# GAP-LAB-CUHK-SZ/GaussReg

Measured on AMD Instinct MI355X. Metric: GS views/sec @1M pts 640x480 (+ radius_neighbors Mpts/sec, see radius_neighbors), higher is better.
Workload: dtype f32; 1 GPU; diff_gaussian_rasterization forward: 1000000 synthetic Gaussians (SH deg 3), 640x480, 32 views per step per GPU (configs[1]); gaussians=1000000, width=640, height=480, parallelism=per-view sharding x1

## Files before the change

### gaussreg_amd/_lib.py

```python
import ctypes
import os
import re

_HERE = os.path.dirname(os.path.abspath(__file__))
LIB_PATH = os.path.join(_HERE, "lib", "libgaussreg_hip.so")
HEADER_PATH = os.path.join(_HERE, "..", "include", "gaussreg_hip.h")
TRAIN_HEADER_PATH = os.path.join(_HERE, "..", "include", "gaussreg_hip_train.h")
MATCH_TRAIN_HEADER_PATH = os.path.join(_HERE, "..", "include", "gaussreg_hip_train_matching.h")
BACKBONE_TRAIN_HEADER_PATH = os.path.join(_HERE, "..", "include", "gaussreg_hip_train_backbone.h")

_lib = None

c_void = ctypes.c_void_p
c_f32 = ctypes.c_float


class RasterView(ctypes.Structure):
    _fields_ = [("image_height", ctypes.c_int32), ("image_width", ctypes.c_int32),
                ("tanfovx", c_f32), ("tanfovy", c_f32), ("bg", c_f32 * 3), ("scale_modifier", c_f32),
                ("viewmatrix", c_f32 * 16), ("projmatrix", c_f32 * 16), ("campos", c_f32 * 3),
                ("sh_degree", ctypes.c_int32), ("prefiltered", ctypes.c_int32), ("debug", ctypes.c_int32)]


class GsAdamGroup(ctypes.Structure):
    _fields_ = [("param", c_void), ("grad", c_void), ("exp_avg", c_void), ("exp_avg_sq", c_void),
                ("lr", ctypes.c_double), ("K", ctypes.c_int32)]


class GsDensifyGroup(ctypes.Structure):
    _fields_ = [("src_param", c_void), ("dst_param", c_void), ("src_exp_avg", c_void), ("dst_exp_avg", c_void),
                ("src_exp_avg_sq", c_void), ("dst_exp_avg_sq", c_void), ("K", ctypes.c_int32), ("role", ctypes.c_int32)]

# ... 35 lines not shown
        if r is None:
            raise ValueError(f"gaussreg_hip.h: cannot parse the return type '{ret}' of {name}")
        restype = None if r.groups() == ("void", "") else _ctype(r.group(1), r.group(2), f"the return type of {name}")
        argtypes = []
        for arg in ([] if args in ("", "void") else args.split(",")):
            a = re.fullmatch(_TYPE + r"(?:\s*(\*)\s*|\s+)\w+", arg.strip())
            if a is None:
                raise ValueError(f"gaussreg_hip.h: cannot parse the argument '{arg.strip()}' of {name}")
            argtypes.append(_ctype(a.group(1), a.group(2) or "", f"argument '{arg.strip()}' of {name}"))
        if name in signatures:
            raise ValueError(f"gaussreg_hip.h: {name} is declared twice")
        signatures[name] = (restype, argtypes)
    return signatures, defines


with open(HEADER_PATH) as _f:
    SIGNATURES, DEFINES = parse_header(_f.read())
with open(TRAIN_HEADER_PATH) as _f:
    TRAIN_SIGNATURES, TRAIN_DEFINES = parse_header(_f.read())
with open(MATCH_TRAIN_HEADER_PATH) as _f:
    MATCH_TRAIN_SIGNATURES, MATCH_TRAIN_DEFINES = parse_header(_f.read())
with open(BACKBONE_TRAIN_HEADER_PATH) as _f:
    BACKBONE_TRAIN_SIGNATURES, BACKBONE_TRAIN_DEFINES = parse_header(_f.read())

GR_PENDING = DEFINES["GR_PENDING"]
GR_RETRY_FULL = DEFINES["GR_RETRY_FULL"]
GR_RETRY_BIN = DEFINES["GR_RETRY_BIN"]
GS_ADAM_MAX_GROUPS = DEFINES["GR_GS_ADAM_MAX_GROUPS"]
GS_KNN_MAX_K = DEFINES["GR_GS_KNN_MAX_K"]
GS_DENSIFY_CARRIED, GS_DENSIFY_XYZ, GS_DENSIFY_SCALING = (DEFINES["GR_GS_DENSIFY_" + r] for r in ("CARRIED", "XYZ", "SCALING"))


class HipLibraryError(RuntimeError):
    pass


def lib():
    global _lib
    if _lib is None:
        import torch
        if not os.path.exists(LIB_PATH):
            raise HipLibraryError(
                f"{LIB_PATH} is missing: build it with `python -m gaussreg_amd.build` "
                "(there is no CPU fallback for the gaussreg_amd ops)")
        L = ctypes.CDLL(LIB_PATH)
        for name, (res, args) in (list(SIGNATURES.items()) + list(TRAIN_SIGNATURES.items())
                                   + list(MATCH_TRAIN_SIGNATURES.items()) + list(BACKBONE_TRAIN_SIGNATURES.items())):
            fn = getattr(L, name)
            fn.restype = res
            fn.argtypes = args
        _lib = L
    return _lib


def check(rc, allow=()):
    if rc != 0 and rc not in allow:
        msg = lib().gr_last_error()
        raise RuntimeError("gaussreg_hip: " + (msg.decode() if msg else f"error {rc}"))
    return rc


def tensor_stamp(tensors):
    out = []
    for t in tensors:
        if t.is_inference():
            return None
        out.append((t.data_ptr(), t._version))
    return tuple(out)


# ... 87 lines not shown
```

### gaussreg_amd/build.py

```python
import concurrent.futures
import os
import subprocess
import sys

HERE = os.path.dirname(os.path.abspath(__file__))
CSRC = os.path.join(HERE, "csrc")
LIBDIR = os.path.join(HERE, "lib")
OBJDIR = os.path.join(LIBDIR, "obj")
LIB = os.path.join(LIBDIR, "libgaussreg_hip.so")

HIPCC = os.environ.get("HIPCC", "/opt/rocm/bin/hipcc")
FLAGS = ["--offload-arch=gfx950", "-O3", "-std=c++17", "-fPIC", "-ffp-contract=off", "-Wall",
         "-Wno-unused-function", "-Wno-unused-result"]


def sources():
    return sorted(f for f in os.listdir(CSRC) if f.endswith(".hip"))


def _stale(out, deps):
    if not os.path.exists(out):
        return True
    t = os.path.getmtime(out)
    return any(os.path.getmtime(d) > t for d in deps)


def build(force=False, verbose=False):
    os.makedirs(OBJDIR, exist_ok=True)
    headers = [os.path.join(CSRC, f) for f in os.listdir(CSRC) if f.endswith((".hpp", ".h"))]
    headers += [os.path.join(HERE, "..", "include", h) for h in ("gaussreg_hip.h", "gaussreg_hip_train.h",
                                                                 "gaussreg_hip_train_matching.h",
                                                                 "gaussreg_hip_train_backbone.h")]
    jobs = []
    objs = []
    for src in sources():
        s = os.path.join(CSRC, src)
        o = os.path.join(OBJDIR, src[:-4] + ".o")
        objs.append(o)
        if force or _stale(o, [s] + headers):
            jobs.append([HIPCC] + FLAGS + ["-c", s, "-o", o])

    def run(cmd):
        if verbose:
            print(" ".join(cmd), flush=True)
        r = subprocess.run(cmd, stdout=subprocess.PIPE, stderr=subprocess.STDOUT, text=True)
        return cmd, r.returncode, r.stdout

    if jobs:
        with concurrent.futures.ThreadPoolExecutor(max_workers=min(8, len(jobs))) as ex:
            for cmd, rc, out in ex.map(run, jobs):
                if rc != 0:
                    raise RuntimeError("hipcc failed: %s\n%s" % (" ".join(cmd), out))
                if verbose and out.strip():
                    print(out)
    if force or jobs or _stale(LIB, objs):
# ... 10 lines not shown
```

### gaussreg_amd/csrc/preprocess_body.hpp

```cpp
#ifndef GR_PREPROCESS_BODY_OK
#error "preprocess_body.hpp is the body of the two preprocess kernels of rasterizer.hip"
#endif
static_assert(std::is_same<decltype(WAVE_MM), const bool>::value, "the including kernel defines `constexpr bool WAVE_MM`");
  if (LATE && blockIdx.x == 0 && threadIdx.x < (int)(sizeof(DevView) / 4))
    reinterpret_cast<float*>(const_cast<DevView*>(views))[threadIdx.x] = reinterpret_cast<const float*>(&cam1)[threadIdx.x];
  __shared__ float4 s_sh[(SH16 && !LATE) ? WAVE * SH_ROW : 1];
  __shared__ float4 s_rec[256 / WAVE][4 * REC_PLANE];
  __shared__ int s_mm[WAVE_MM ? 1 : 2][2][256 / WAVE];
  int i = blockIdx.x * blockDim.x + threadIdx.x;
  float shr[SH16 ? 48 : 1];
  if (SH16 && !LATE) {
    const int g0 = blockIdx.x * 256;
    const int n_here = min(256, P - g0);
    const float4* src = reinterpret_cast<const float4*>(shs + (int64_t)g0 * 48);
#pragma unroll 1
    for (int w = 0; w < 256 / WAVE; ++w) {
      const int lim = min(WAVE, n_here - w * WAVE) * 12;
#pragma unroll
      for (int u = 0; u < 3; ++u) {
        const int f = threadIdx.x + u * 256;
        if (f < lim) {
          const int g = f / 12, j = f - g * 12;
          s_sh[g * SH_ROW + j] = src[w * WAVE * 12 + f];
        }
      }
      __syncthreads();
      if ((int)threadIdx.x / WAVE == w && i < P) {
#pragma unroll
// ... 14 lines not shown
  i = min(i, P - 1);
  const float p[3] = {means3D[3 * (int64_t)i], means3D[3 * (int64_t)i + 1], means3D[3 * (int64_t)i + 2]};
  const float opacity = opacities[i];
  float c6[6];
  if (HAS_COV) {
#pragma unroll
    for (int k = 0; k < 6; ++k) c6[k] = cov3D_precomp[6 * (int64_t)i + k];
  }
  const int gx = (W + TILE - 1) / TILE, gy = (H + TILE - 1) / TILE;
  const float* sh = HAS_SH ? shs + (int64_t)i * M * 3 : nullptr;
  float cpre[3] = {0.f, 0.f, 0.f};
  if (!HAS_SH) {
#pragma unroll
    for (int k = 0; k < 3; ++k) cpre[k] = colors_precomp[3 * (int64_t)i + k];
  }
  float4* wrec = s_rec[threadIdx.x / WAVE];
  float mod_prev = 0.f;
  bool have_cov = HAS_COV;
  for (int v = 0; v < V; ++v) {
    const DevView& cam = LATE ? cam1 : views[v];
    const int64_t o = (int64_t)v * P + i;
    int out_radius = 0;
    uint32_t out_field = 0u, out_rect = 0u;
    float out_depth = 0.f, out_sxx = INFINITY, out_syy = INFINITY, out_kc = 0.f;
    float2 out_xy = make_float2(0.f, 0.f);
    float4 out_co = make_float4(0.f, 0.f, 0.f, 0.f);
    bool shade = false;
    float rgb[3] = {0.f, 0.f, 0.f};
    float pv[3];
    xform4x3(cam.view, p, pv);
    if (pv[2] > 0.2f) {
      float ph[4];
      xform4x4(cam.proj, p, ph);
      const float pw = 1.0f / (ph[3] + 0.0000001f);
      const float pprojx = ph[0] * pw, pprojy = ph[1] * pw;
      if (!HAS_COV && (!have_cov || cam.scale_mod != mod_prev)) {
        float sc[3], rot[4];
#pragma unroll
        for (int k = 0; k < 3; ++k) sc[k] = scales[3 * (int64_t)i + k];
#pragma unroll
        for (int k = 0; k < 4; ++k) rot[k] = rotations[4 * (int64_t)i + k];
        cov3d_from_scale_rot(sc, cam.scale_mod, rot, c6);
        have_cov = true;
        mod_prev = cam.scale_mod;
      }
      float cv[3];
      cov2d(pv, cam.fx, cam.fy, cam.tanx, cam.tany, c6, cam.view, cv);
      const float det = cv[0] * cv[2] - cv[1] * cv[1];
      if (det != 0.0f) {
        const float det_inv = 1.f / det;
        const float mid = 0.5f * (cv[0] + cv[2]);
        const float sq = sqrtf(fmaxf(0.1f, mid * mid - det));
        const float l1 = mid + sq, l2 = mid - sq;
        const float my_radius = ceilf(3.f * sqrtf(fmaxf(l1, l2)));
        const float px = ((pprojx + 1.0f) * (float)W - 1.0f) * 0.5f;
        const float py = ((pprojy + 1.0f) * (float)H - 1.0f) * 0.5f;
        int rmin[2], rmax[2];
        get_rect(px, py, (int)my_radius, gx, gy, rmin, rmax);
        const int ntile = (rmax[0] - rmin[0]) * (rmax[1] - rmin[1]);
        if (ntile != 0) {
          shade = true;
          if (HAS_SH && SH16 && LATE) {
            const float4* s4 = reinterpret_cast<const float4*>(shs + (int64_t)i * 48);
#pragma unroll
            for (int jj = 0; jj < 12; ++jj) {
              const float4 t4 = s4[jj];
              shr[4 * jj] = t4.x;
              shr[4 * jj + 1] = t4.y;
              shr[4 * jj + 2] = t4.z;
              shr[4 * jj + 3] = t4.w;
            }
            sh_to_rgb(D, p, cam.campos, [&](int k, int c) { return shr[k * 3 + c]; }, rgb);
          }
          out_depth = pv[2];
          out_radius = (int)my_radius;
          out_xy = make_float2(px, py);
          out_co = make_float4(cv[2] * det_inv, -cv[1] * det_inv, cv[0] * det_inv, opacity);
          const bool cullable = det > 0.0f && l2 >= 0.29f && l1 < 1.0e4f;
          const float kc = cullable ? 1.001f / (0.5f / l1 - 2.0e-6f) : INFINITY;
          out_kc = kc;
          if (cullable) {
            out_sxx = 2.0f * cv[0] * 1.004f;
            out_syy = 2.0f * cv[2] * 1.004f;
            const float pcm = __logf(255.0f * opacity) + 2.0e-3f;
            if (pcm > 0.0f) {
              const float cp = pcm + 2.0e-6f * (pcm * kc);
              const float hx = sqrtf(2.0f * cp * cv[0]) * 1.001f + 1.0e-2f;
              const float hy = sqrtf(2.0f * cp * cv[2]) * 1.001f + 1.0e-2f;
              const float xlo = ceilf(px - hx), xhi = floorf(px + hx), ylo = ceilf(py - hy), yhi = floorf(py + hy);
              if (xlo > -1.0e6f && xhi < 1.0e6f && ylo > -1.0e6f && yhi < 1.0e6f) {
                rmin[0] = max(rmin[0], (int)floorf(xlo / (float)TILE));
                rmin[1] = max(rmin[1], (int)floorf(ylo / (float)TILE));
                rmax[0] = min(rmax[0], (int)floorf(xhi / (float)TILE) + 1);
                rmax[1] = min(rmax[1], (int)floorf(yhi / (float)TILE) + 1);
                if (rmax[0] < rmin[0]) rmax[0] = rmin[0];
                if (rmax[1] < rmin[1]) rmax[1] = rmin[1];
              }
            }
          }
          uint32_t dk = __float_as_uint(out_depth) - KEY_DEPTH_BASE;
          if (dk >= (1u << KEY_DEPTH_BITS)) {
            dk = (1u << KEY_DEPTH_BITS) - 1;
            if (LATE) *far_flag = far_seq; else atomicOr(far_flag, 1);
          }
          out_field = dk;
          out_rect = pack_rect(rmin, rmax);
        }
      }
    }
    if (valid) {
      __builtin_nontemporal_store(out_radius, radii + o);
      dfield[o] = out_field;
      rect_raw[o] = out_rect;
    }
    wrec[0 * REC_PLANE + lane] = make_float4(out_xy.x, out_xy.y, out_sxx, out_syy);
    wrec[1 * REC_PLANE + lane] = out_co;
    wrec[3 * REC_PLANE + lane] = make_float4(__int_as_float(out_radius), out_depth, 0.f, 0.f);
    if (WAVE_MM) {
      const uint32_t fld = valid ? out_field : 0u;
      const int mn = wave_min_i32_dpp(fld != 0u ? (int)fld : 0x7fffffff), mx = wave_max_i32_dpp((int)fld);
      const int wave_id = __builtin_amdgcn_readfirstlane((int)(blockIdx.x * (256 / WAVE) + threadIdx.x / WAVE));
      if (lane == 0) key_mm[(int64_t)v * (gridDim.x * (256 / WAVE)) + wave_id] = make_int2(mn, mx);
      __builtin_amdgcn_fence(__ATOMIC_RELEASE, "wavefront");
      __builtin_amdgcn_wave_barrier();
      __builtin_amdgcn_fence(__ATOMIC_ACQUIRE, "wavefront");
    } else if (key_mm != nullptr) {
      const uint32_t fld = valid ? out_field : 0u;
      const int mn = wave_min_i32_dpp(fld != 0u ? (int)fld : 0x7fffffff), mx = wave_max_i32_dpp((int)fld);
      if (lane == 0) s_mm[v & 1][0][threadIdx.x / WAVE] = mn, s_mm[v & 1][1][threadIdx.x / WAVE] = mx;
      __syncthreads();
      if (threadIdx.x == 0) {
        int bmn = 0x7fffffff, bmx = 0;
#pragma unroll
        for (int w = 0; w < 256 / WAVE; ++w) bmn = min(bmn, s_mm[v & 1][0][w]), bmx = max(bmx, s_mm[v & 1][1][w]);
        key_mm[(int64_t)v * gridDim.x + blockIdx.x] = make_int2(bmn, bmx);
      }
    }
    if (shade && !(HAS_SH && SH16 && LATE)) {
      if (HAS_SH) {
        if (SH16) sh_to_rgb(D, p, cam.campos, [&](int k, int c) { return shr[k * 3 + c]; }, rgb);
        else sh_to_rgb(D, p, cam.campos, [&](int k, int c) { return sh[k * 3 + c]; }, rgb);
      } else {
        rgb[0] = cpre[0]; rgb[1] = cpre[1]; rgb[2] = cpre[2];
      }
    }
    wrec[2 * REC_PLANE + lane] = make_float4(rgb[0], rgb[1], rgb[2], out_kc);
    const unsigned long long vis = __ballot(valid && out_radius > 0);
    __builtin_amdgcn_fence(__ATOMIC_RELEASE, "wavefront");
    __builtin_amdgcn_wave_barrier();
    __builtin_amdgcn_fence(__ATOMIC_ACQUIRE, "wavefront");
    float4* wout = rec + 4 * ((int64_t)v * P + wave_first);
#pragma unroll
    for (int k = 0; k < 4; ++k) {
      const int rl = 16 * k + lane / 4;
      const float4 piece = wrec[(lane & 3) * REC_PLANE + rl];
      if ((vis >> rl) & 1ull) {
        typedef float pre_f4 __attribute__((ext_vector_type(4)));
        __builtin_nontemporal_store(pre_f4{piece.x, piece.y, piece.z, piece.w}, reinterpret_cast<pre_f4*>(wout + 4 * rl + (lane & 3)));
      }
    }
    __builtin_amdgcn_fence(__ATOMIC_RELEASE, "wavefront");
    __builtin_amdgcn_wave_barrier();
    __builtin_amdgcn_fence(__ATOMIC_ACQUIRE, "wavefront");
  }
```

### gaussreg_amd/csrc/raster_shared.hpp

```cpp
#pragma once

#include "common.hpp"

namespace gr {
namespace {

constexpr int TILE = 16;
constexpr int BLOCK = TILE * TILE;
constexpr int MAX_VIEWS = 64;

struct DevView {
  float view[16];
  float proj[16];
  float campos[3];
  float tanx, tany;
  float fx, fy;
  float scale_mod;
  float bg[3];
};

__device__ __constant__ float SH_C0 = 0.28209479177387814f;
__device__ __constant__ float SH_C1 = 0.4886025119029199f;
__device__ __constant__ float SH_C2[5] = {1.0925484305920792f, -1.0925484305920792f,
                                          0.31539156525252005f, -1.0925484305920792f,
// ... 11 lines not shown
  const float nf = tm - MAGIC;
  const float f = fmaf(x, L2E, -nf);
  float p = 1.3264815788716078e-3f;
  p = fmaf(p, f, 9.671512059867382e-3f);
  p = fmaf(p, f, 5.550733581185341e-2f);
  p = fmaf(p, f, 2.4022242426872253e-1f);
  p = fmaf(p, f, 6.931470036506653e-1f);
  p = fmaf(p, f, 1.0f);
  return __uint_as_float(__float_as_uint(p) + (__float_as_uint(tm) << 23));
}

__device__ __forceinline__ void xform4x3(const float* M, const float* p, float* o) {
  o[0] = fmaf(M[0], p[0], fmaf(M[4], p[1], fmaf(M[8], p[2], M[12])));
  o[1] = fmaf(M[1], p[0], fmaf(M[5], p[1], fmaf(M[9], p[2], M[13])));
  o[2] = fmaf(M[2], p[0], fmaf(M[6], p[1], fmaf(M[10], p[2], M[14])));
}
__device__ __forceinline__ void xform4x4(const float* M, const float* p, float* o) {
  o[0] = fmaf(M[0], p[0], fmaf(M[4], p[1], fmaf(M[8], p[2], M[12])));
  o[1] = fmaf(M[1], p[0], fmaf(M[5], p[1], fmaf(M[9], p[2], M[13])));
  o[2] = fmaf(M[2], p[0], fmaf(M[6], p[1], fmaf(M[10], p[2], M[14])));
  o[3] = fmaf(M[3], p[0], fmaf(M[7], p[1], fmaf(M[11], p[2], M[15])));
}

__device__ __forceinline__ void cov3d_from_scale_rot(const float* sc, float mod, const float* q,
                                                     float* c6) {
  const float s0 = mod * sc[0], s1 = mod * sc[1], s2 = mod * sc[2];
  const float r = q[0], x = q[1], y = q[2], z = q[3];
  float R[3][3];
  R[0][0] = 1.f - 2.f * (y * y + z * z);
  R[0][1] = 2.f * (x * y - r * z);
  R[0][2] = 2.f * (x * z + r * y);
  R[1][0] = 2.f * (x * y + r * z);
  R[1][1] = 1.f - 2.f * (x * x + z * z);
  R[1][2] = 2.f * (y * z - r * x);
  R[2][0] = 2.f * (x * z - r * y);
  R[2][1] = 2.f * (y * z + r * x);
  R[2][2] = 1.f - 2.f * (x * x + y * y);
  float M[3][3];
#pragma unroll
  for (int i = 0; i < 3; ++i) {
    M[0][i] = s0 * R[i][0];
    M[1][i] = s1 * R[i][1];
    M[2][i] = s2 * R[i][2];
  }
#define GR_SIG(i, j) fmaf(M[0][i], M[0][j], fmaf(M[1][i], M[1][j], M[2][i] * M[2][j]))
  c6[0] = GR_SIG(0, 0);
  c6[1] = GR_SIG(0, 1);
  c6[2] = GR_SIG(0, 2);
  c6[3] = GR_SIG(1, 1);
  c6[4] = GR_SIG(1, 2);
  c6[5] = GR_SIG(2, 2);
#undef GR_SIG
}

__device__ __forceinline__ void cov2d(const float* t_in, float fx, float fy, float tanx, float tany,
                                      const float* c6, const float* V, float* out3) {
  float t[3] = {t_in[0], t_in[1], t_in[2]};
  const float limx = 1.3f * tanx, limy = 1.3f * tany;
  const float txtz = t[0] / t[2], tytz = t[1] / t[2];
  t[0] = fminf(limx, fmaxf(-limx, txtz)) * t[2];
  t[1] = fminf(limy, fmaxf(-limy, tytz)) * t[2];
  const float J00 = fx / t[2];
  const float J02 = -(fx * t[0]) / (t[2] * t[2]);
  const float J11 = fy / t[2];
  const float J12 = -(fy * t[1]) / (t[2] * t[2]);
  float A0[3], A1[3];
#pragma unroll
  for (int j = 0; j < 3; ++j) {
    A0[j] = fmaf(J00, V[j * 4 + 0], J02 * V[j * 4 + 2]);
    A1[j] = fmaf(J11, V[j * 4 + 1], J12 * V[j * 4 + 2]);
  }
  const float S[3][3] = {{c6[0], c6[1], c6[2]}, {c6[1], c6[3], c6[4]}, {c6[2], c6[4], c6[5]}};
  float B0[3], B1[3];
#pragma unroll
  for (int k = 0; k < 3; ++k) {
    B0[k] = fmaf(S[k][0], A0[0], fmaf(S[k][1], A0[1], S[k][2] * A0[2]));
    B1[k] = fmaf(S[k][0], A1[0], fmaf(S[k][1], A1[1], S[k][2] * A1[2]));
  }
  out3[0] = fmaf(A0[0], B0[0], fmaf(A0[1], B0[1], A0[2] * B0[2])) + 0.3f;
  out3[1] = fmaf(A1[0], B0[0], fmaf(A1[1], B0[1], A1[2] * B0[2]));
  out3[2] = fmaf(A1[0], B1[0], fmaf(A1[1], B1[1], A1[2] * B1[2])) + 0.3f;
}

template <typename ShLoad>
__device__ __forceinline__ void sh_to_rgb(int deg, const float* pos, const float* campos,
                                          ShLoad S, float* rgb) {
  const float dx = pos[0] - campos[0], dy = pos[1] - campos[1], dz = pos[2] - campos[2];
  const float len = sqrtf(dx * dx + dy * dy + dz * dz);
  const float x = dx / len, y = dy / len, z = dz / len;
#pragma unroll
  for (int c = 0; c < 3; ++c) {
    float res = SH_C0 * S(0, c);
    if (deg > 0) {
      res = res - SH_C1 * y * S(1, c) + SH_C1 * z * S(2, c) - SH_C1 * x * S(3, c);
      if (deg > 1) {
        const float xx = x * x, yy = y * y, zz = z * z, xy = x * y, yz = y * z, xz = x * z;
        res = res + SH_C2[0] * xy * S(4, c) + SH_C2[1] * yz * S(5, c) +
              SH_C2[2] * (2.0f * zz - xx - yy) * S(6, c) + SH_C2[3] * xz * S(7, c) +
              SH_C2[4] * (xx - yy) * S(8, c);
        if (deg > 2) {
          res = res + SH_C3[0] * y * (3.0f * xx - yy) * S(9, c) + SH_C3[1] * xy * z * S(10, c) +
                SH_C3[2] * y * (4.0f * zz - xx - yy) * S(11, c) +
                SH_C3[3] * z * (2.0f * zz - 3.0f * xx - 3.0f * yy) * S(12, c) +
                SH_C3[4] * x * (4.0f * zz - xx - yy) * S(13, c) +
                SH_C3[5] * z * (xx - yy) * S(14, c) + SH_C3[6] * x * (xx - 3.0f * yy) * S(15, c);
        }
      }
    }
    res += 0.5f;
    rgb[c] = fmaxf(res, 0.0f);
  }
}

struct Geom {
  float4* rec;
  uint32_t* dfield;
  uint32_t* rect_raw;
  uint64_t* keys_a;
  uint64_t* keys_b;
  int32_t* order_a;
  int32_t* order_b;
  uint32_t* rects;
  uint16_t* chunk_cnt;
  uint32_t* seg_off;
  int32_t* chunk_total;
  int32_t* chunk_max;
  void* ds_table;
  size_t ds_table_bytes;
  int2* key_mm;
  int32_t* nvis;
  int32_t* totals;
  DevView* views;
  int32_t* scan_ws;
  size_t bytes;
// ... 50 lines not shown
```

### gaussreg_amd/csrc/rasterizer.hip

```cpp
#include <algorithm>
#include <type_traits>
#include <vector>

#include <atomic>

#include "raster_shared.hpp"

namespace gr {
namespace {

static_assert(TILE == RASTER_TILE, "get_rect / rect_decode (common.hpp) are written for this tile size");


constexpr int KEY_DEPTH_BITS = 27;
constexpr uint32_t KEY_DEPTH_BASE = 0x3E000000u;

__device__ __forceinline__ uint32_t pack_rect(const int* rmin, const int* rmax) {
  const int w = rmax[0] - rmin[0], h = rmax[1] - rmin[1];
  if (w > 63 || h > 63 || rmin[0] > 126 || rmin[1] > 126) return RECT_MARKER26;
  return (uint32_t)rmin[0] | ((uint32_t)rmin[1] << 7) | ((uint32_t)w << 14) | ((uint32_t)h << 20);
}

constexpr int REC_PLANE = 66;
constexpr int SH_ROW = 13;

template <bool HAS_SH, bool HAS_COV, bool SH16, bool LATE>
__global__ __launch_bounds__(256) void preprocess_kernel(
    int P, int D, int M, int V, const DevView* __restrict__ views, const float* __restrict__ means3D,
    const float* __restrict__ shs, const float* __restrict__ colors_precomp,
    const float* __restrict__ opacities, const float* __restrict__ scales,
    const float* __restrict__ rotations, const float* __restrict__ cov3D_precomp, int W, int H,
    int32_t* __restrict__ radii, float4* __restrict__ rec, uint32_t* __restrict__ dfield,
    uint32_t* __restrict__ rect_raw, int32_t* __restrict__ far_flag, DevView cam1, int far_seq,
    int2* __restrict__ key_mm) {
  constexpr bool WAVE_MM = false;
#define GR_PREPROCESS_BODY_OK
#include "preprocess_body.hpp"
#undef GR_PREPROCESS_BODY_OK
}

template <bool HAS_SH, bool HAS_COV, bool SH16>
__global__ __launch_bounds__(256) void preprocess_many_kernel(
    int P, int D, int M, int V, const DevView* __restrict__ views, const float* __restrict__ means3D,
    const float* __restrict__ shs, const float* __restrict__ colors_precomp,
// ... 883 lines not shown
      if (r <= prev) atomicOr(bad, 2);
      prev = r;
    }
  }
}

}
}

namespace gr {
namespace {
std::atomic<int> g_frames[64];

bool verify_this_frame() {
  static const bool always = getenv("GR_RASTER_VERIFY") && getenv("GR_RASTER_VERIFY")[0] == '1';
  if (lds_atomics_lane_ordered_state() != 1) return always;
  int dev = 0;
  if (hipGetDevice(&dev) != hipSuccess || dev < 0 || dev >= 64) dev = 63;
  const int f = g_frames[dev].load();
  return always || f < 3 || (f & 255) == 0;
}

thread_local int g_bucket_cooldown = 0;
constexpr int BUCKET_COOLDOWN_FRAMES = 256;
bool bucket_sort_allowed(bool possible) {
  if (!possible) return false;
  if (g_bucket_cooldown == 0) return true;
  --g_bucket_cooldown;
  return false;
}
void bucket_sort_overflowed() { g_bucket_cooldown = BUCKET_COOLDOWN_FRAMES; }

void frame_done() {
  int dev = 0;
  if (hipGetDevice(&dev) != hipSuccess || dev < 0 || dev >= 64) dev = 63;
  g_frames[dev].fetch_add(1);
}

template <typename F>
int device_check(hipStream_t stream, F&& launch_check, int* h_flag) {
  int* d_bad = nullptr;
  GR_HIP(hipMallocAsync(reinterpret_cast<void**>(&d_bad), sizeof(int), stream));
  GR_HIP(hipMemsetAsync(d_bad, 0, sizeof(int), stream));
  launch_check(d_bad);
  GR_HIP(hipMemcpyAsync(h_flag, d_bad, sizeof(int), hipMemcpyDeviceToHost, stream));
  GR_HIP(hipStreamSynchronize(stream));
// ... 127 lines not shown
  Geom g = carve_geom(geom, P, num_views, tiles);
  if (!geom || geom_bytes < g.bytes) {
    set_error("raster geometry buffer too small: need %zu bytes, got %zu", g.bytes, geom_bytes);
    return GR_ERR_WORKSPACE;
  }
  const dim3 blk(256), grd((unsigned)((P + 255) / 256));
  const bool sh16 = shs != nullptr && M == 16 && (reinterpret_cast<uintptr_t>(shs) % 16 == 0);
  const bool cam_in_args = sh16 && num_views == 1 && defer_ev != nullptr && defer_ev->mail != nullptr &&
                           (P + BIN_CHUNK - 1) / BIN_CHUNK <= SCAN_SINGLE_ROW;
  DevView cam1;
  memset(&cam1, 0, sizeof(cam1));
  int far_seq = 1;
  if (sh16 && num_views == 1) fill_view(cam1, h_views[0]);
  if (cam_in_args) {
    far_seq = defer_ev->seq;
  } else {
    rc = upload_views(h_views, num_views, g.totals + 2 * num_views, stream);
    if (rc != GR_OK) return rc;
  }
  if (defer_ev != nullptr) defer_ev->far_seq = far_seq;
  const bool msd_possible = depth_sort_msd_possible(P, num_views, KEY_DEPTH_BITS);
  const bool msd = msd_possible && (defer_ev != nullptr ? defer_ev->bucket_sort : bucket_sort_allowed(true));
  int2* const mm_out = msd ? g.key_mm : nullptr;
#define GR_PRE(SH, COV, S16)                                                                       \
  if (S16 && num_views == 1)                                                                       \
    hipLaunchKernelGGL((preprocess_kernel<SH, COV, S16, S16>), grd, blk, 0, stream, (int)P, D, M, num_views, \
                       g.views, means3D, shs, colors_precomp, opacities, scales, rotations,        \
                       cov3D_precomp, W, H, radii, g.rec, g.dfield, g.rect_raw, g.totals + 2 * num_views, cam1, far_seq, \
                       mm_out);                                                                    \
  else if (msd && num_views > 4)                                                                   \
    hipLaunchKernelGGL((preprocess_many_kernel<SH, COV, S16>), grd, blk, 0, stream, (int)P, D, M, num_views, \
                       g.views, means3D, shs, colors_precomp, opacities, scales, rotations,        \
                       cov3D_precomp, W, H, radii, g.rec, g.dfield, g.rect_raw, g.totals + 2 * num_views, cam1, far_seq, \
                       mm_out);                                                                    \
  else                                                                                             \
  hipLaunchKernelGGL((preprocess_kernel<SH, COV, S16, false>), grd, blk, 0, stream, (int)P, D, M, num_views, \
                     g.views, means3D, shs, colors_precomp, opacities, scales, rotations,          \
                     cov3D_precomp, W, H, radii, g.rec, g.dfield, g.rect_raw, g.totals + 2 * num_views, cam1, far_seq, \
                     mm_out)
  auto run_preprocess = [&]() {
    KernelTimer timer("raster_preprocess", stream);
    if (shs && cov3D_precomp) { if (sh16) GR_PRE(true, true, true); else GR_PRE(true, true, false); }
    else if (shs) { if (sh16) GR_PRE(true, false, true); else GR_PRE(true, false, false); }
    else if (cov3D_precomp) GR_PRE(false, true, false);
    else GR_PRE(false, false, false);
  };
  run_preprocess();
  GR_LAUNCH_CHECK();
  int32_t* tot = static_cast<int32_t*>(pinned_scratch(1, sizeof(int32_t) * (2 * num_views + 2)));
  GR_REQUIRE(tot != nullptr, "pinned read-back buffer could not be allocated");
  const int nchunk = (int)((P + BIN_CHUNK - 1) / BIN_CHUNK);
  int32_t h_chunk_max = 0;
  auto sort_and_count = [&](int key_bits, bool buckets = true) -> int {
    bool totals_sorted = false;
    {
      KernelTimer timer("raster_depth_sort", stream);
      const bool msd_now = msd && buckets && key_bits == KEY_DEPTH_BITS;
      const bool self_seg = msd_now && defer_ev != nullptr && defer_ev->mail != nullptr && nchunk <= SCAN_SINGLE_ROW &&
                            num_views <= 4;
// ... 300 lines not shown
extern "C" int gr_raster_render_aux(int64_t P, const gr_raster_view* h_views, int num_views,
                                    const int64_t* h_num_rendered, const void* geom, size_t geom_bytes,
                                    void* bin, size_t bin_bytes, float* out_color, float* out_depth, float* out_alpha,
                                    float* out_state, int flags, void* stream_) {
  GR_REQUIRE(out_depth != nullptr && out_alpha != nullptr, "out_depth / out_alpha is null");
  return render_impl(P, h_views, num_views, h_num_rendered, geom, geom_bytes, bin, bin_bytes, out_color, flags, -1,
                     static_cast<hipStream_t>(stream_), nullptr, out_state != nullptr, out_depth, out_alpha, out_state);
}

namespace gr {
namespace {
struct Pending {
  bool open;
  int64_t P;
  int num_views;
  int64_t entries;
  Deferred d;
  hipStream_t stream;
};
thread_local Pending g_pending{false, 0, 0, 0, Deferred{nullptr, nullptr, 0, 0, false, false, false}, nullptr};
}
}

extern "C" int gr_raster_debug_bucket_cooldown(int set) {
  const int left = gr::g_bucket_cooldown;
  if (set >= 0) gr::g_bucket_cooldown = set;
  return left;
}

extern "C" int gr_raster_forward_finish(int64_t* h_num_rendered) {
  using namespace gr;
  GR_REQUIRE(g_pending.open, "gr_raster_forward_finish: no split gr_raster_forward is open on this thread");
  GR_REQUIRE(h_num_rendered != nullptr, "h_num_rendered is null");
  Pending p = g_pending;
  g_pending.open = false;
  bool far_depth = false, bucket_overflow = false;
  int rc = preprocess_collect(p.P, p.num_views, h_num_rendered, &far_depth, p.d, p.stream, &bucket_overflow);
  if (rc != GR_OK) return rc;
  if (bucket_overflow) bucket_sort_overflowed();
  int64_t R = 0;
  for (int v = 0; v < p.num_views; ++v) R += h_num_rendered[v];
  if (far_depth) return GR_RETRY_FULL;
  return R <= p.entries ? GR_OK : GR_RETRY_BIN;
}

extern "C" int gr_raster_forward(int64_t P, int M, const float* means3D, const float* shs, const float* colors_precomp,
// ... 71 lines not shown
```

Baseline: 13820 views/s.

## Use wave-uniform fast reciprocal/sqrt paths in preprocess with cold exact fallback

```diff
diff --git a/gaussreg_amd/_lib.py b/gaussreg_amd/_lib.py
--- a/gaussreg_amd/_lib.py
+++ b/gaussreg_amd/_lib.py
@@ -8,6 +8,7 @@
 TRAIN_HEADER_PATH = os.path.join(_HERE, "..", "include", "gaussreg_hip_train.h")
 MATCH_TRAIN_HEADER_PATH = os.path.join(_HERE, "..", "include", "gaussreg_hip_train_matching.h")
 BACKBONE_TRAIN_HEADER_PATH = os.path.join(_HERE, "..", "include", "gaussreg_hip_train_backbone.h")
+DEBUG_HEADER_PATH = os.path.join(_HERE, "..", "include", "gaussreg_hip_debug.h")
 
 _lib = None
 
@@ -89,6 +90,8 @@
     MATCH_TRAIN_SIGNATURES, MATCH_TRAIN_DEFINES = parse_header(_f.read())
 with open(BACKBONE_TRAIN_HEADER_PATH) as _f:
     BACKBONE_TRAIN_SIGNATURES, BACKBONE_TRAIN_DEFINES = parse_header(_f.read())
+with open(DEBUG_HEADER_PATH) as _f:
+    DEBUG_SIGNATURES, DEBUG_DEFINES = parse_header(_f.read())
 
 GR_PENDING = DEFINES["GR_PENDING"]
 GR_RETRY_FULL = DEFINES["GR_RETRY_FULL"]
@@ -112,7 +115,8 @@
                 "(there is no CPU fallback for the gaussreg_amd ops)")
         L = ctypes.CDLL(LIB_PATH)
         for name, (res, args) in (list(SIGNATURES.items()) + list(TRAIN_SIGNATURES.items())
-                                   + list(MATCH_TRAIN_SIGNATURES.items()) + list(BACKBONE_TRAIN_SIGNATURES.items())):
+                                   + list(MATCH_TRAIN_SIGNATURES.items()) + list(BACKBONE_TRAIN_SIGNATURES.items())
+                                   + list(DEBUG_SIGNATURES.items())):
             fn = getattr(L, name)
             fn.restype = res
             fn.argtypes = args
diff --git a/gaussreg_amd/build.py b/gaussreg_amd/build.py
--- a/gaussreg_amd/build.py
+++ b/gaussreg_amd/build.py
@@ -30,7 +30,7 @@
     headers = [os.path.join(CSRC, f) for f in os.listdir(CSRC) if f.endswith((".hpp", ".h"))]
     headers += [os.path.join(HERE, "..", "include", h) for h in ("gaussreg_hip.h", "gaussreg_hip_train.h",
                                                                  "gaussreg_hip_train_matching.h",
-                                                                 "gaussreg_hip_train_backbone.h")]
+                                                                 "gaussreg_hip_train_backbone.h", "gaussreg_hip_debug.h")]
     jobs = []
     objs = []
     for src in sources():
diff --git a/gaussreg_amd/csrc/preprocess_body.hpp b/gaussreg_amd/csrc/preprocess_body.hpp
--- a/gaussreg_amd/csrc/preprocess_body.hpp
+++ b/gaussreg_amd/csrc/preprocess_body.hpp
@@ -4,6 +4,8 @@
 static_assert(std::is_same<decltype(WAVE_MM), const bool>::value, "the including kernel defines `constexpr bool WAVE_MM`");
   if (LATE && blockIdx.x == 0 && threadIdx.x < (int)(sizeof(DevView) / 4))
     reinterpret_cast<float*>(const_cast<DevView*>(views))[threadIdx.x] = reinterpret_cast<const float*>(&cam1)[threadIdx.x];
+  const bool plain_div = (D & GR_PRE_PLAIN_DIV) != 0;
+  const int deg = D & (GR_PRE_PLAIN_DIV - 1);
   __shared__ float4 s_sh[(SH16 && !LATE) ? WAVE * SH_ROW : 1];
   __shared__ float4 s_rec[256 / WAVE][4 * REC_PLANE];
   __shared__ int s_mm[WAVE_MM ? 1 : 2][2][256 / WAVE];
@@ -64,39 +66,41 @@
     const int64_t o = (int64_t)v * P + i;
     int out_radius = 0;
     uint32_t out_field = 0u, out_rect = 0u;
-    float out_depth = 0.f, out_sxx = INFINITY, out_syy = INFINITY, out_kc = 0.f;
-    float2 out_xy = make_float2(0.f, 0.f);
-    float4 out_co = make_float4(0.f, 0.f, 0.f, 0.f);
+    float out_kc;
     bool shade = false;
-    float rgb[3] = {0.f, 0.f, 0.f};
     float pv[3];
     xform4x3(cam.view, p, pv);
+    pv[0] = lone(pv[0]), pv[1] = lone(pv[1]), pv[2] = lone(pv[2]);
     if (pv[2] > 0.2f) {
       float ph[4];
       xform4x4(cam.proj, p, ph);
+      ph[0] = lone(ph[0]), ph[1] = lone(ph[1]), ph[3] = lone(ph[3]);
       const float pw = 1.0f / (ph[3] + 0.0000001f);
-      const float pprojx = ph[0] * pw, pprojy = ph[1] * pw;
+      const float pprojx = lone(ph[0] * pw), pprojy = lone(ph[1] * pw);
       if (!HAS_COV && (!have_cov || cam.scale_mod != mod_prev)) {
         float sc[3], rot[4];
 #pragma unroll
         for (int k = 0; k < 3; ++k) sc[k] = scales[3 * (int64_t)i + k];
 #pragma unroll
         for (int k = 0; k < 4; ++k) rot[k] = rotations[4 * (int64_t)i + k];
-        cov3d_from_scale_rot(sc, cam.scale_mod, rot, c6);
+        GR_COLD_BEGIN("+v"(sc[0]), "+v"(sc[1]), "+v"(sc[2]), "+v"(rot[0]), "+v"(rot[1]), "+v"(rot[2]), "+v"(rot[3]));
+        cov3d_from_scale_rot<true>(sc, cam.scale_mod, rot, c6);
         have_cov = true;
         mod_prev = cam.scale_mod;
+        GR_COLD_END("+v"(c6[0]), "+v"(c6[1]), "+v"(c6[2]), "+v"(c6[3]), "+v"(c6[4]), "+v"(c6[5]));
       }
       float cv[3];
-      cov2d(pv, cam.fx, cam.fy, cam.tanx, cam.tany, c6, cam.view, cv);
-      const float det = cv[0] * cv[2] - cv[1] * cv[1];
+      cov2d(pv, cam.fx, cam.fy, cam.tanx, cam.tany, c6, cam.view, cv, plain_div);
+      const float det = lone(cv[0] * cv[2]) - lone(cv[1] * cv[1]);
       if (det != 0.0f) {
         const float det_inv = 1.f / det;
         const float mid = 0.5f * (cv[0] + cv[2]);
-        const float sq = sqrtf(fmaxf(0.1f, mid * mid - det));
+        const float sq = sqrt_in_range(fmaxf(0.1f, mid * mid - det), true, plain_div);
         const float l1 = mid + sq, l2 = mid - sq;
-        const float my_radius = ceilf(3.f * sqrtf(fmaxf(l1, l2)));
-        const float px = ((pprojx + 1.0f) * (float)W - 1.0f) * 0.5f;
-        const float py = ((pprojy + 1.0f) * (float)H - 1.0f) * 0.5f;
+        const float lmax = fmaxf(l1, l2);
+        const float my_radius = ceilf(3.f * sqrt_in_range(lmax, lmax >= 0x1p-96f, plain_div));
+        const float px = lone(lone(lone(lone(pprojx + 1.0f) * (float)W) - 1.0f) * 0.5f);
+        const float py = lone(lone(lone(lone(pprojy + 1.0f) * (float)H) - 1.0f) * 0.5f);
         int rmin[2], rmax[2];
         get_rect(px, py, (int)my_radius, gx, gy, rmin, rmax);
         const int ntile = (rmax[0] - rmin[0]) * (rmax[1] - rmin[1]);
@@ -112,23 +116,23 @@
               shr[4 * jj + 2] = t4.z;
               shr[4 * jj + 3] = t4.w;
             }
-            sh_to_rgb(D, p, cam.campos, [&](int k, int c) { return shr[k * 3 + c]; }, rgb);
-          }
-          out_depth = pv[2];
+          }
+          float out_sxx = INFINITY, out_syy = INFINITY;
           out_radius = (int)my_radius;
-          out_xy = make_float2(px, py);
-          out_co = make_float4(cv[2] * det_inv, -cv[1] * det_inv, cv[0] * det_inv, opacity);
+          const float out_depth = pv[2];
           const bool cullable = det > 0.0f && l2 >= 0.29f && l1 < 1.0e4f;
           const float kc = cullable ? 1.001f / (0.5f / l1 - 2.0e-6f) : INFINITY;
           out_kc = kc;
           if (cullable) {
-            out_sxx = 2.0f * cv[0] * 1.004f;
-            out_syy = 2.0f * cv[2] * 1.004f;
+            out_sxx = lone(lone(2.0f * cv[0]) * 1.004f);
+            out_syy = lone(lone(2.0f * cv[2]) * 1.004f);
             const float pcm = __logf(255.0f * opacity) + 2.0e-3f;
             if (pcm > 0.0f) {
               const float cp = pcm + 2.0e-6f * (pcm * kc);
-              const float hx = sqrtf(2.0f * cp * cv[0]) * 1.001f + 1.0e-2f;
-              const float hy = sqrtf(2.0f * cp * cv[2]) * 1.001f + 1.0e-2f;
+              const float hx2 = lone(2.0f * cp * cv[0]), hy2 = lone(2.0f * cp * cv[2]);
+              const bool h_ok = fminf(hx2, hy2) >= 0x1p-96f;
+              const float hx = sqrt_in_range(hx2, h_ok, plain_div) * 1.001f + 1.0e-2f;
+              const float hy = sqrt_in_range(hy2, h_ok, plain_div) * 1.001f + 1.0e-2f;
               const float xlo = ceilf(px - hx), xhi = floorf(px + hx), ylo = ceilf(py - hy), yhi = floorf(py + hy);
               if (xlo > -1.0e6f && xhi < 1.0e6f && ylo > -1.0e6f && yhi < 1.0e6f) {
                 rmin[0] = max(rmin[0], (int)floorf(xlo / (float)TILE));
@@ -147,6 +151,14 @@
           }
           out_field = dk;
           out_rect = pack_rect(rmin, rmax);
+          wrec[0 * REC_PLANE + lane] = make_float4(px, py, out_sxx, out_syy);
+          wrec[1 * REC_PLANE + lane] = make_float4(lone(cv[2] * det_inv), lone(-cv[1] * det_inv), lone(cv[0] * det_inv), opacity);
+          wrec[3 * REC_PLANE + lane] = make_float4(__int_as_float(out_radius), pv[2], 0.f, 0.f);
+          if (HAS_SH && SH16 && LATE) {
+            float rgb[3];
+            sh_to_rgb_fwd(deg, p, cam.campos, [&](int k, int c) { return shr[k * 3 + c]; }, rgb, plain_div);
+            wrec[2 * REC_PLANE + lane] = make_float4(rgb[0], rgb[1], rgb[2], out_kc);
+          }
         }
       }
     }
@@ -155,9 +167,6 @@
       dfield[o] = out_field;
       rect_raw[o] = out_rect;
     }
-    wrec[0 * REC_PLANE + lane] = make_float4(out_xy.x, out_xy.y, out_sxx, out_syy);
-    wrec[1 * REC_PLANE + lane] = out_co;
-    wrec[3 * REC_PLANE + lane] = make_float4(__int_as_float(out_radius), out_depth, 0.f, 0.f);
     if (WAVE_MM) {
       const uint32_t fld = valid ? out_field : 0u;
       const int mn = wave_min_i32_dpp(fld != 0u ? (int)fld : 0x7fffffff), mx = wave_max_i32_dpp((int)fld);
@@ -179,14 +188,15 @@
       }
     }
     if (shade && !(HAS_SH && SH16 && LATE)) {
+      float rgb[3];
       if (HAS_SH) {
-        if (SH16) sh_to_rgb(D, p, cam.campos, [&](int k, int c) { return shr[k * 3 + c]; }, rgb);
-        else sh_to_rgb(D, p, cam.campos, [&](int k, int c) { return sh[k * 3 + c]; }, rgb);
+        if (SH16) sh_to_rgb_fwd(deg, p, cam.campos, [&](int k, int c) { return shr[k * 3 + c]; }, rgb, plain_div);
+        else sh_to_rgb_fwd(deg, p, cam.campos, [&](int k, int c) { return sh[k * 3 + c]; }, rgb, plain_div);
       } else {
         rgb[0] = cpre[0]; rgb[1] = cpre[1]; rgb[2] = cpre[2];
       }
-    }
-    wrec[2 * REC_PLANE + lane] = make_float4(rgb[0], rgb[1], rgb[2], out_kc);
+      wrec[2 * REC_PLANE + lane] = make_float4(rgb[0], rgb[1], rgb[2], out_kc);
+    }
     const unsigned long long vis = __ballot(valid && out_radius > 0);
     __builtin_amdgcn_fence(__ATOMIC_RELEASE, "wavefront");
     __builtin_amdgcn_wave_barrier();
diff --git a/gaussreg_amd/csrc/raster_shared.hpp b/gaussreg_amd/csrc/raster_shared.hpp
--- a/gaussreg_amd/csrc/raster_shared.hpp
+++ b/gaussreg_amd/csrc/raster_shared.hpp
@@ -57,28 +57,38 @@
   o[3] = fmaf(M[3], p[0], fmaf(M[7], p[1], fmaf(M[11], p[2], M[15])));
 }
 
+#define GR_COLD_BEGIN(...) asm volatile("; gr_cold_begin" : __VA_ARGS__)
+#define GR_COLD_END(...) asm volatile("; gr_cold_end" : __VA_ARGS__)
+
+__device__ __forceinline__ float lone(float x) {
+  asm("" : "+v"(x));
+  return x;
+}
+
+template <bool ALONE = false>
 __device__ __forceinline__ void cov3d_from_scale_rot(const float* sc, float mod, const float* q,
                                                      float* c6) {
   const float s0 = mod * sc[0], s1 = mod * sc[1], s2 = mod * sc[2];
   const float r = q[0], x = q[1], y = q[2], z = q[3];
+  auto w = [](float v) { return ALONE ? lone(v) : v; };
   float R[3][3];
-  R[0][0] = 1.f - 2.f * (y * y + z * z);
-  R[0][1] = 2.f * (x * y - r * z);
-  R[0][2] = 2.f * (x * z + r * y);
-  R[1][0] = 2.f * (x * y + r * z);
-  R[1][1] = 1.f - 2.f * (x * x + z * z);
-  R[1][2] = 2.f * (y * z - r * x);
-  R[2][0] = 2.f * (x * z - r * y);
-  R[2][1] = 2.f * (y * z + r * x);
-  R[2][2] = 1.f - 2.f * (x * x + y * y);
+  R[0][0] = w(1.f - 2.f * (w(y * y) + z * z));
+  R[0][1] = w(2.f * (w(x * y) - r * z));
+  R[0][2] = w(2.f * (w(x * z) + r * y));
+  R[1][0] = w(2.f * (w(x * y) + r * z));
+  R[1][1] = w(1.f - 2.f * (w(x * x) + z * z));
+  R[1][2] = w(2.f * (w(y * z) - r * x));
+  R[2][0] = w(2.f * (w(x * z) - r * y));
+  R[2][1] = w(2.f * (w(y * z) + r * x));
+  R[2][2] = w(1.f - 2.f * (w(x * x) + y * y));
   float M[3][3];
 #pragma unroll
   for (int i = 0; i < 3; ++i) {
-    M[0][i] = s0 * R[i][0];
-    M[1][i] = s1 * R[i][1];
-    M[2][i] = s2 * R[i][2];
-  }
-#define GR_SIG(i, j) fmaf(M[0][i], M[0][j], fmaf(M[1][i], M[1][j], M[2][i] * M[2][j]))
+    M[0][i] = w(s0 * R[i][0]);
+    M[1][i] = w(s1 * R[i][1]);
+    M[2][i] = w(s2 * R[i][2]);
+  }
+#define GR_SIG(i, j) w(fmaf(M[0][i], M[0][j], fmaf(M[1][i], M[1][j], w(M[2][i] * M[2][j]))))
   c6[0] = GR_SIG(0, 0);
   c6[1] = GR_SIG(0, 1);
   c6[2] = GR_SIG(0, 2);
@@ -88,33 +98,81 @@
 #undef GR_SIG
 }
 
+__device__ __forceinline__ bool wave_all(bool ok) { return __builtin_amdgcn_ballot_w64(!ok) == 0ull; }
+
+template <int N>
+__device__ __forceinline__ void div_shared(const float (&n)[N], float d, float (&q)[N]) {
+  const float r0 = __builtin_amdgcn_rcpf(d);
+  const float r1 = lone(fmaf(lone(fmaf(-d, r0, 1.0f)), r0, r0));
+#pragma unroll
+  for (int k = 0; k < N; ++k) {
+    const float m0 = lone(n[k] * r1);
+    const float m1 = lone(fmaf(lone(fmaf(-d, m0, n[k])), r1, m0));
+    q[k] = lone(fmaf(lone(fmaf(-d, m1, n[k])), r1, m1));
+  }
+}
+
+__device__ __forceinline__ float sqrt_in_range(float x, bool in_range, bool plain) {
+  if (!plain && wave_all(in_range)) {
+    const float s = lone(__builtin_amdgcn_sqrtf(x));
+    const float dn = __uint_as_float(__float_as_uint(s) - 1u), up = __uint_as_float(__float_as_uint(s) + 1u);
+    const float vp = lone(fmaf(-dn, s, x)), vs = lone(fmaf(-up, s, x));
+    const float r = vp <= 0.0f ? dn : s;
+    return lone(vs > 0.0f ? up : r);
+  }
+  float y = x, r;
+  GR_COLD_BEGIN("+v"(y));
+  r = sqrtf(y);
+  GR_COLD_END("+v"(r));
+  return r;
+}
+
 __device__ __forceinline__ void cov2d(const float* t_in, float fx, float fy, float tanx, float tany,
-                                      const float* c6, const float* V, float* out3) {
+                                      const float* c6, const float* V, float* out3, bool plain_div) {
   float t[3] = {t_in[0], t_in[1], t_in[2]};
   const float limx = 1.3f * tanx, limy = 1.3f * tany;
-  const float txtz = t[0] / t[2], tytz = t[1] / t[2];
-  t[0] = fminf(limx, fmaxf(-limx, txtz)) * t[2];
-  t[1] = fminf(limy, fmaxf(-limy, tytz)) * t[2];
-  const float J00 = fx / t[2];
-  const float J02 = -(fx * t[0]) / (t[2] * t[2]);
-  const float J11 = fy / t[2];
-  const float J12 = -(fy * t[1]) / (t[2] * t[2]);
+  const float hi = fmaxf(fmaxf(fabsf(t[0]), fabsf(t[1])), fabsf(t[2])), lo = fminf(fminf(fabsf(t[0]), fabsf(t[1])), fabsf(t[2]));
+  const bool cam_ok = fminf(fx, fy) >= 0x1p-16f && fmaxf(fx, fy) <= 0x1p16f && fminf(limx, limy) >= 0x1p-10f &&
+                      fmaxf(limx, limy) <= 0x1p10f;
+  float J00, J02, J11, J12;
+  if (!plain_div && cam_ok && wave_all(lo >= 0x1p-16f && hi <= 0x1p16f)) {
+    const float n1[4] = {t[0], t[1], fx, fy};
+    float q1[4];
+    div_shared(n1, t[2], q1);
+    t[0] = fminf(limx, fmaxf(-limx, q1[0])) * t[2];
+    t[1] = fminf(limy, fmaxf(-limy, q1[1])) * t[2];
+    const float n2[2] = {-lone(fx * t[0]), -lone(fy * t[1])};
+    float q2[2];
+    div_shared(n2, t[2] * t[2], q2);
+    J00 = q1[2], J11 = q1[3], J02 = q2[0], J12 = q2[1];
+  } else {
+    GR_COLD_BEGIN("+v"(t[0]), "+v"(t[1]), "+v"(t[2]));
+    const float txtz = t[0] / t[2], tytz = t[1] / t[2];
+    t[0] = fminf(limx, fmaxf(-limx, txtz)) * t[2];
+    t[1] = fminf(limy, fmaxf(-limy, tytz)) * t[2];
+    J00 = fx / t[2];
+    J02 = -lone(fx * t[0]) / (t[2] * t[2]);
+    J11 = fy / t[2];
+    J12 = -lone(fy * t[1]) / (t[2] * t[2]);
+    GR_COLD_END("+v"(J00), "+v"(J02), "+v"(J11), "+v"(J12));
+  }
+  J00 = lone(J00), J02 = lone(J02), J11 = lone(J11), J12 = lone(J12);
   float A0[3], A1[3];
 #pragma unroll
   for (int j = 0; j < 3; ++j) {
-    A0[j] = fmaf(J00, V[j * 4 + 0], J02 * V[j * 4 + 2]);
-    A1[j] = fmaf(J11, V[j * 4 + 1], J12 * V[j * 4 + 2]);
+    A0[j] = lone(fmaf(J00, V[j * 4 + 0], J02 * V[j * 4 + 2]));
+    A1[j] = lone(fmaf(J11, V[j * 4 + 1], J12 * V[j * 4 + 2]));
   }
   const float S[3][3] = {{c6[0], c6[1], c6[2]}, {c6[1], c6[3], c6[4]}, {c6[2], c6[4], c6[5]}};
   float B0[3], B1[3];
 #pragma unroll
   for (int k = 0; k < 3; ++k) {
-    B0[k] = fmaf(S[k][0], A0[0], fmaf(S[k][1], A0[1], S[k][2] * A0[2]));
-    B1[k] = fmaf(S[k][0], A1[0], fmaf(S[k][1], A1[1], S[k][2] * A1[2]));
-  }
-  out3[0] = fmaf(A0[0], B0[0], fmaf(A0[1], B0[1], A0[2] * B0[2])) + 0.3f;
-  out3[1] = fmaf(A1[0], B0[0], fmaf(A1[1], B0[1], A1[2] * B0[2]));
-  out3[2] = fmaf(A1[0], B1[0], fmaf(A1[1], B1[1], A1[2] * B1[2])) + 0.3f;
+    B0[k] = lone(fmaf(S[k][0], A0[0], fmaf(S[k][1], A0[1], S[k][2] * A0[2])));
+    B1[k] = lone(fmaf(S[k][0], A1[0], fmaf(S[k][1], A1[1], S[k][2] * A1[2])));
+  }
+  out3[0] = lone(fmaf(A0[0], B0[0], fmaf(A0[1], B0[1], A0[2] * B0[2])) + 0.3f);
+  out3[1] = lone(fmaf(A1[0], B0[0], fmaf(A1[1], B0[1], A1[2] * B0[2])));
+  out3[2] = lone(fmaf(A1[0], B1[0], fmaf(A1[1], B1[1], A1[2] * B1[2])) + 0.3f);
 }
 
 template <typename ShLoad>
@@ -145,6 +203,63 @@
     res += 0.5f;
     rgb[c] = fmaxf(res, 0.0f);
   }
+}
+
+template <typename ShLoad>
+__device__ __forceinline__ void sh_to_rgb_fwd(int deg, const float* pos, const float* campos, ShLoad S, float* rgb,
+                                              bool plain_div) {
+  const float dx = lone(pos[0] - campos[0]), dy = lone(pos[1] - campos[1]), dz = lone(pos[2] - campos[2]);
+  const float len2 = lone(lone(dx * dx) + lone(dy * dy)) + lone(dz * dz);
+  float x, y, z, len;
+  if (!plain_div && wave_all(fminf(fminf(fabsf(dx), fabsf(dy)), fabsf(dz)) >= 0x1p-40f &&
+                             fmaxf(fmaxf(fabsf(dx), fabsf(dy)), fabsf(dz)) <= 0x1p39f)) {
+    len = sqrt_in_range(len2, true, false);
+    const float n[3] = {dx, dy, dz};
+    float q[3];
+    div_shared(n, len, q);
+    x = q[0], y = q[1], z = q[2];
+  } else {
+    float l = len2;
+    GR_COLD_BEGIN("+v"(l));
+    l = sqrtf(l);
+    x = dx / l, y = dy / l, z = dz / l;
+    GR_COLD_END("+v"(x), "+v"(y), "+v"(z));
+  }
+  x = lone(x), y = lone(y), z = lone(z);
+  float res[3];
+#pragma unroll
+  for (int c = 0; c < 3; ++c) res[c] = lone(SH_C0 * S(0, c));
+  if (deg > 0) {
+    const float b1 = lone(SH_C1 * y), b2 = lone(SH_C1 * z), b3 = lone(SH_C1 * x);
+#pragma unroll
+    for (int c = 0; c < 3; ++c) res[c] = lone(lone(lone(res[c] - lone(b1 * S(1, c))) + lone(b2 * S(2, c))) - lone(b3 * S(3, c)));
+    if (deg > 1) {
+      const float xx = lone(x * x), yy = lone(y * y), zz = lone(z * z), xy = lone(x * y), yz = lone(y * z), xz = lone(x * z);
+      const float b2nd[5] = {lone(SH_C2[0] * xy), lone(SH_C2[1] * yz), lone(SH_C2[2] * (2.0f * zz - xx - yy)),
+                             lone(SH_C2[3] * xz), lone(SH_C2[4] * (xx - yy))};
+#pragma unroll
+      for (int c = 0; c < 3; ++c) {
+#pragma unroll
+        for (int k = 0; k < 5; ++k) res[c] = lone(res[c] + lone(b2nd[k] * S(4 + k, c)));
+      }
+      if (deg > 2) {
+        const float b3rd[7] = {lone(lone(SH_C3[0] * y) * (3.0f * xx - yy)),
+                               lone(lone(SH_C3[1] * xy) * z),
+                               lone(lone(SH_C3[2] * y) * (4.0f * zz - xx - yy)),
+                               lone(lone(SH_C3[3] * z) * (2.0f * zz - 3.0f * xx - 3.0f * yy)),
+                               lone(lone(SH_C3[4] * x) * (4.0f * zz - xx - yy)),
+                               lone(lone(SH_C3[5] * z) * (xx - yy)),
+                               lone(lone(SH_C3[6] * x) * (xx - 3.0f * yy))};
+#pragma unroll
+        for (int c = 0; c < 3; ++c) {
+#pragma unroll
+          for (int k = 0; k < 7; ++k) res[c] = lone(res[c] + lone(b3rd[k] * S(9 + k, c)));
+        }
+      }
+    }
+  }
+#pragma unroll
+  for (int c = 0; c < 3; ++c) rgb[c] = lone(fmaxf(lone(res[c] + 0.5f), 0.0f));
 }
 
 struct Geom {
diff --git a/gaussreg_amd/csrc/rasterizer.hip b/gaussreg_amd/csrc/rasterizer.hip
--- a/gaussreg_amd/csrc/rasterizer.hip
+++ b/gaussreg_amd/csrc/rasterizer.hip
@@ -20,6 +20,8 @@
   if (w > 63 || h > 63 || rmin[0] > 126 || rmin[1] > 126) return RECT_MARKER26;
   return (uint32_t)rmin[0] | ((uint32_t)rmin[1] << 7) | ((uint32_t)w << 14) | ((uint32_t)h << 20);
 }
+
+constexpr int GR_PRE_PLAIN_DIV = 0x100;
 
 constexpr int REC_PLANE = 66;
 constexpr int SH_ROW = 13;
@@ -949,6 +951,7 @@
 }
 
 thread_local int g_bucket_cooldown = 0;
+std::atomic<int> g_plain_division{0};
 constexpr int BUCKET_COOLDOWN_FRAMES = 256;
 bool bucket_sort_allowed(bool possible) {
   if (!possible) return false;
@@ -1122,19 +1125,20 @@
   const bool msd_possible = depth_sort_msd_possible(P, num_views, KEY_DEPTH_BITS);
   const bool msd = msd_possible && (defer_ev != nullptr ? defer_ev->bucket_sort : bucket_sort_allowed(true));
   int2* const mm_out = msd ? g.key_mm : nullptr;
+  const int Dk = D | (g_plain_division ? GR_PRE_PLAIN_DIV : 0);
 #define GR_PRE(SH, COV, S16)                                                                       \
   if (S16 && num_views == 1)                                                                       \
-    hipLaunchKernelGGL((preprocess_kernel<SH, COV, S16, S16>), grd, blk, 0, stream, (int)P, D, M, num_views, \
+    hipLaunchKernelGGL((preprocess_kernel<SH, COV, S16, S16>), grd, blk, 0, stream, (int)P, Dk, M, num_views, \
                        g.views, means3D, shs, colors_precomp, opacities, scales, rotations,        \
                        cov3D_precomp, W, H, radii, g.rec, g.dfield, g.rect_raw, g.totals + 2 * num_views, cam1, far_seq, \
                        mm_out);                                                                    \
   else if (msd && num_views > 4)                                                                   \
-    hipLaunchKernelGGL((preprocess_many_kernel<SH, COV, S16>), grd, blk, 0, stream, (int)P, D, M, num_views, \
+    hipLaunchKernelGGL((preprocess_many_kernel<SH, COV, S16>), grd, blk, 0, stream, (int)P, Dk, M, num_views, \
                        g.views, means3D, shs, colors_precomp, opacities, scales, rotations,        \
                        cov3D_precomp, W, H, radii, g.rec, g.dfield, g.rect_raw, g.totals + 2 * num_views, cam1, far_seq, \
                        mm_out);                                                                    \
   else                                                                                             \
-  hipLaunchKernelGGL((preprocess_kernel<SH, COV, S16, false>), grd, blk, 0, stream, (int)P, D, M, num_views, \
+  hipLaunchKernelGGL((preprocess_kernel<SH, COV, S16, false>), grd, blk, 0, stream, (int)P, Dk, M, num_views, \
                      g.views, means3D, shs, colors_precomp, opacities, scales, rotations,          \
                      cov3D_precomp, W, H, radii, g.rec, g.dfield, g.rect_raw, g.totals + 2 * num_views, cam1, far_seq, \
                      mm_out)
@@ -1481,6 +1485,12 @@
 }
 }
 
+extern "C" int gr_raster_debug_plain_division(int set) {
+  const int was = gr::g_plain_division;
+  if (set >= 0) gr::g_plain_division = set != 0;
+  return was;
+}
+
 extern "C" int gr_raster_debug_bucket_cooldown(int set) {
   const int left = gr::g_bucket_cooldown;
   if (set >= 0) gr::g_bucket_cooldown = set;
diff --git a/include/gaussreg_hip_debug.h b/include/gaussreg_hip_debug.h
--- /dev/null
+++ b/include/gaussreg_hip_debug.h
@@ -0,0 +1,17 @@
+#ifndef GAUSSREG_HIP_DEBUG_H_
+#define GAUSSREG_HIP_DEBUG_H_
+
+#include <stddef.h>
+#include <stdint.h>
+
+#ifdef __cplusplus
+extern "C" {
+#endif
+
+int gr_raster_debug_plain_division(int set);
+
+#ifdef __cplusplus
+}
+#endif
+
+#endif
```

Result: no change. 13900 views/s, median of 6 (+0.6%).
